# ethz-asl/laser_slam

Measured on NVIDIA H100. Metric: ICP registrations/s (131072-pt scan vs 524288-pt map, 30 iterations), higher is better.
Workload: dtype f32

## Files before the change

laser_slam_b200/csrc/ls_api.cu:

```cuda
#include <cmath>
#include <cstdarg>
#include <cstddef>
#include <cstdio>
#include <cstdlib>
#include <cstring>
#include <string>
#include <utility>
#include <vector>

#include "../../include/ls_b200.h"
#include "ls_filters.cuh"
#include "ls_kernels.cuh"
#include "ls_occupancy.cuh"

using namespace ls;

#define LS_VERSION 100

struct Workspace {
  cudaStream_t stream = nullptr;
  cudaEvent_t ev0 = nullptr, ev1 = nullptr, ev2 = nullptr, ev_launch = nullptr;
  int n_cap = 0, m_cap = 0, cells_cap = 0, tab_cap = 0, hist_cap = 0;
  BuildArrays A{};
  BuildState* bs = nullptr;
  float4* rd = nullptr;
  int* pos = nullptr;
  float4 *vq = nullptr, *vpts = nullptr;
  float* d2 = nullptr;
  int* ids = nullptr;
  float* d2_out = nullptr;
  IcpWork* work = nullptr;
  float* T_hist = nullptr;
  BuildJob* job_host = nullptr;
  BuildJob* job_dev = nullptr;
  IcpWork* h_work = nullptr;
  Grid* h_grid = nullptr;
  IcpProblem hp;
  bool stream_dirty = false;
};

struct ls_ctx {
  int device = 0;
  int sm_count = 0;
  int icp_ctas = 0;
  int icp_ctas_max = 0;
  std::string err;
  uint64_t launches = 0;
  std::vector<Workspace*> ws;
  IcpProblem* probs_dev = nullptr;
  IcpProblem* probs_host = nullptr;
  BuildJob* jobs_dev = nullptr;
  BuildJob* jobs_host = nullptr;
  IcpWork* work_pool = nullptr;
  float4* reading = nullptr;
  float4 *ref_stage = nullptr, *ref_nrm_stage = nullptr;
  int reading_cap = 0, ref_cap = 0;
  float* nrm_raw = nullptr;
  size_t nrm_raw_cap = 0;
  float* T0_dev = nullptr;
  unsigned char* xbuf = nullptr;
  unsigned char* xpeer[8] = {nullptr, nullptr, nullptr, nullptr, nullptr, nullptr, nullptr, nullptr};
  int shard_rank = 0, shard_count = 1;
  bool xconnected = false;
  unsigned int xflag_base = 0;
  bool pending = false;
  int pending_batch = 0;
  std::vector<int> pending_ws;
  std::vector<int> pending_n;
  std::vector<float> pending_T0;
  std::vector<std::pair<const ls_map*, int>> pending_slots;
  lsf::ChainBuffers chain;
};
constexpr int kMaxBatch = 160;

struct ls_scan_slot {
  float4* pts = nullptr;
// ... 180 lines not shown
  const int cap = batch > 1 ? ctx->sm_count * 2 : ctx->sm_count * 8;
  const int pb = blocks_for(m_max, 256, cap);
  reset_build_kernel<<<dim3(1, B), 32, 0, st>>>(jobs_dev);
  LAUNCH_CHECK();
  assemble_kernel<<<dim3(pb, B), 256, 0, st>>>(jobs_dev);
  LAUNCH_CHECK();
  setup_kernel<<<dim3(1, B), 32, 0, st>>>(jobs_dev, r.cell, r.max_cells, r.split);
  LAUNCH_CHECK();
  count0_kernel<<<dim3(pb, B), 256, 0, st>>>(jobs_dev);
  LAUNCH_CHECK();
  const int tiles = (r.max_cells + kScanTile - 1) / kScanTile;
  scan_reduce_kernel<<<dim3(tiles, B), kScanThreads, 0, st>>>(jobs_dev);
  LAUNCH_CHECK();
  scan_apply_kernel<<<dim3(tiles, B), kScanThreads, 0, st>>>(jobs_dev);
  LAUNCH_CHECK();
  pyramid1_kernel<<<dim3(blocks_for(r.max_cells / 16 + 1, 256, batch > 1 ? ctx->sm_count : ctx->sm_count * 4), B), 256, 0, st>>>(jobs_dev);
  LAUNCH_CHECK();
  pyramid_up_kernel<<<dim3(1, B), 1024, 0, st>>>(jobs_dev);
  LAUNCH_CHECK();
  count1_kernel<<<dim3(pb, B), 256, 0, st>>>(jobs_dev);
  LAUNCH_CHECK();
  tables_kernel<<<dim3(cap, B), 256, 0, st>>>(jobs_dev);
  LAUNCH_CHECK();
  scatter_kernel<<<dim3(pb, B), 256, 0, st>>>(jobs_dev);
  LAUNCH_CHECK();
  return LS_OK;
}

int launch_reading_sort(ls_ctx* ctx, const BuildJob* jobs_dev, int batch, int n_max, const Resolved& r, cudaStream_t st) {
  const unsigned int B = (unsigned int)batch;
  const int cap = batch > 1 ? ctx->sm_count * 2 : ctx->sm_count * 8;
  const int qb = blocks_for(n_max, 256, cap);
  const int scan_tiles = (r.max_cells + kScanTile - 1) / kScanTile;
  reading_kernel<<<dim3(qb, B), 256, 0, st>>>(jobs_dev);
  LAUNCH_CHECK();
  q_count_kernel<<<dim3(qb, B), 256, 0, st>>>(jobs_dev);
  LAUNCH_CHECK();
  q_tables_kernel<<<dim3(cap, B), 256, 0, st>>>(jobs_dev);
  LAUNCH_CHECK();
  q_scan_reduce_kernel<<<dim3(scan_tiles, B), kScanThreads, 0, st>>>(jobs_dev);
  LAUNCH_CHECK();
  q_scan_apply_kernel<<<dim3(scan_tiles, B), kScanThreads, 0, st>>>(jobs_dev);
  LAUNCH_CHECK();
  q_scatter_kernel<<<dim3(qb, B), 256, 0, st>>>(jobs_dev);
  LAUNCH_CHECK();
  return LS_OK;
}

int enqueue_build(ls_ctx* ctx, Workspace* w, const Parts& parts, const Resolved& r, const float* T0_host) {
  fill_job(w, parts, T0_host, nullptr, 0);
  CU(cudaMemcpyAsync(w->job_dev, w->job_host, sizeof(BuildJob), cudaMemcpyHostToDevice, w->stream));
  return launch_build(ctx, w->job_dev, 1, w->job_host->m, r, w->stream);
}

int upload_normals(ls_ctx* ctx, Workspace* w, const float* normals, int stride, int n, float4* dst) {
  const size_t need = n > 0 ? (stride <= 8 ? (size_t)(n - 1) * (size_t)stride + 3 : (size_t)n * 3) : 0;
  if (need > ctx->nrm_raw_cap) {
    int rc;
// ... 66 lines not shown
  CU(cudaMemcpyAsync(ctx->probs_dev, ctx->probs_host, sizeof(IcpProblem) * (size_t)batch, cudaMemcpyHostToDevice, w0->stream));
  IcpParamsDev dp;
  dp.max_iterations = prm->max_iterations;
  dp.trim_ratio = prm->trim_ratio;
  dp.use_differential = prm->use_differential;
  dp.min_diff_rot = prm->min_diff_rot;
  dp.min_diff_trans = prm->min_diff_trans;
  dp.smooth_length = prm->smooth_length;
  int ctas = ctx->icp_ctas / batch;
  const int need = (n_max + 31) / 32;
  if (ctas > need) ctas = need;
  if (ctas < 1) ctas = 1;
  const IcpProblem* probs = ctx->probs_dev;
  int dynamic = batch > 1 ? 1 : 0;
  void* args[] = {(void*)&probs, (void*)&ctas, (void*)&dp, (void*)&dynamic};
  if (sharded) {
    shard_slice_kernel<<<1, 32, 0, w0->stream>>>(ctx->probs_dev, w0->job_dev, w0->hp.shard_rank, w0->hp.shard_count);
    LAUNCH_CHECK();
  }
  CU(cudaEventRecord(w0->ev_launch, w0->stream));
  CU(cudaLaunchCooperativeKernel((void*)icp_kernel, dim3(ctas * batch), dim3(kIcpThreads), args, kIcpPairBytes, w0->stream));
  ++ctx->launches;
  CU(cudaEventRecord(w0->ev2, w0->stream));
  for (int b = 0; b < batch; ++b) {
    Workspace* w = ctx->ws[b];
    constexpr size_t off = offsetof(IcpWork, T_out);
    CU(cudaMemcpyAsync(reinterpret_cast<char*>(w->h_work) + off, reinterpret_cast<const char*>(w->work) + off,
                       sizeof(IcpWork) - off, cudaMemcpyDeviceToHost, w0->stream));
    CU(cudaMemcpyAsync(w->h_grid, &w->bs->grid, sizeof(Grid), cudaMemcpyDeviceToHost, w0->stream));
  }
  return LS_OK;
}

int fetch_icp(ls_ctx* ctx, Workspace* w, int n, const float T0[16], float T_out[16], ls_icp_stats* stats,
              bool batch_timing = false) {
  const IcpWork& wk = *w->h_work;
  std::memcpy(T_out, wk.T_out, 16 * sizeof(float));
  if (stats) {
    std::memset(stats, 0, sizeof(*stats));
    stats->iterations = wk.iterations;
    stats->converged = wk.converged;
    stats->max_iter_reached = wk.max_iter_reached;
    stats->last_kept = wk.last_kept;
    stats->last_limit = wk.last_limit;
    stats->used_ratio = n > 0 ? (float)wk.last_kept / (float)n : 0.f;
    float ms = 0.f, bms = 0.f, kms = 0.f;
    const Workspace* tw = batch_timing ? ctx->ws[0] : w;
    cudaEventElapsedTime(&ms, tw->ev0, ctx->ws[0]->ev2);
    cudaEventElapsedTime(&bms, tw->ev0, tw->ev1);
    cudaEventElapsedTime(&kms, ctx->ws[0]->ev_launch, ctx->ws[0]->ev2);
    stats->device_ms = ms;
    stats->build_ms = bms;
    stats->icp_ms = kms;
    stats->grid_cells = w->h_grid->n_cells0;
    stats->grid_tables = w->h_grid->n_tab1;
    stats->grid_overflow = w->h_grid->overflow;
  }
  if (wk.status != 0) {
    std::memcpy(T_out, T0, 16 * sizeof(float));
    return fail(ctx, LS_ERR_CONVERGENCE, "ICP: no point to minimise / non-finite transformation");
  }
  return LS_OK;
}

int run_icp(ls_ctx* ctx, const ls_icp_params* prm, const float4* reading_dev, int n, const float T0[16],
            float T_out[16], ls_icp_stats* stats, int32_t* opt_ids, float* opt_d2, float* opt_T_hist) {
  Workspace* w = ctx->ws[0];
  int rc;
  if ((rc = prep_icp(ctx, w, prm, reading_dev, n, T0, opt_ids || opt_d2, opt_T_hist != nullptr))) return rc;
  if ((rc = launch_icp(ctx, prm, 1, n))) return rc;
  if (opt_ids) CU(cudaMemcpyAsync(opt_ids, w->ids, (size_t)n * sizeof(int), cudaMemcpyDeviceToHost, w->stream));
  if (opt_d2) CU(cudaMemcpyAsync(opt_d2, w->d2_out, (size_t)n * sizeof(float), cudaMemcpyDeviceToHost, w->stream));
  if (opt_T_hist)
    CU(cudaMemcpyAsync(opt_T_hist, w->T_hist, (size_t)prm->max_iterations * 16 * sizeof(float), cudaMemcpyDeviceToHost,
                       w->stream));
  CU(cudaStreamSynchronize(w->stream));
  return fetch_icp(ctx, w, n, T0, T_out, stats);
}

bool is_identity16(const float* T) {
  for (int i = 0; i < 16; ++i)
    if (T[i] != ((i % 5 == 0) ? 1.f : 0.f)) return false;
  return true;
}

const ls_scan_slot* find_slot(const ls_map* map, uint64_t id) {
  const ls_scan_slot& s = map->slots[id % (uint64_t)map->capacity];
  return (s.used && s.id == id) ? &s : nullptr;
}

int wait_slot(const ls_scan_slot* s, cudaStream_t consumer) {
  if (s->async && consumer && cudaStreamWaitEvent(consumer, s->ready, 0) != cudaSuccess) return LS_ERR_CUDA;
  return LS_OK;
}

int make_parts(ls_ctx* ctx, const ls_map* map, int n_parts, const uint64_t* part_ids, const float* T_parts, Parts* out,
               cudaStream_t consumer) {
  if (n_parts < 1 || n_parts > kMaxParts) return fail(ctx, LS_ERR_ARG, "n_parts must be in [1,%d]", kMaxParts);
  Parts& parts = *out;
  std::memset(&parts, 0, sizeof(parts));
// ... 11 lines not shown
    parts.identity[p] = is_identity16(T_parts + 16 * p) ? 1 : 0;
    off += s->n;
    if (off > 0x3fffffff) return fail(ctx, LS_ERR_ARG, "sub-map too large");
  }
  parts.offset[n_parts] = (int)off;
  return LS_OK;
}

}

extern "C" {

int ls_b200_version(void) { return LS_VERSION; }

namespace {
Workspace* new_workspace(ls_ctx* ctx, int index) {
  Workspace* w = new Workspace();
  w->work = ctx->work_pool + index;
  w->job_dev = ctx->jobs_dev + index;
  w->job_host = ctx->jobs_host + index;
  bool ok = cudaStreamCreateWithFlags(&w->stream, cudaStreamNonBlocking) == cudaSuccess &&
            cudaEventCreate(&w->ev0) == cudaSuccess && cudaEventCreate(&w->ev1) == cudaSuccess &&
            cudaEventCreate(&w->ev2) == cudaSuccess && cudaEventCreate(&w->ev_launch) == cudaSuccess &&
            cudaMalloc((void**)&w->bs, sizeof(BuildState)) == cudaSuccess &&
            cudaMallocHost((void**)&w->h_work, sizeof(IcpWork)) == cudaSuccess &&
            cudaMallocHost((void**)&w->h_grid, sizeof(Grid)) == cudaSuccess;
  if (!ok) return nullptr;
  return w;
}
void free_workspace(Workspace* w) {
  if (!w) return;
  if (w->stream) cudaStreamSynchronize(w->stream);
  void* bufs[] = {w->A.sub_pts, w->A.sub_nrm, w->A.srt_pts, w->A.srt_nrm, w->A.pkey, w->A.top, w->A.cnt0, w->A.tab1, w->A.cnt1,
                  w->A.tab1_cell, w->A.pyr, w->A.topmask, w->bs, w->rd, w->pos, w->d2,
                  w->ids, w->vq, w->vpts, w->T_hist, w->d2_out, w->A.qkey, w->A.qperm, w->A.rd_s,
                  w->A.qtab_local, w->A.qtab_total, w->A.qtop_start};
  for (void* b : bufs)
    if (b) cudaFree(b);
  if (w->h_work) cudaFreeHost(w->h_work);
  if (w->h_grid) cudaFreeHost(w->h_grid);
  if (w->ev0) cudaEventDestroy(w->ev0);
  if (w->ev1) cudaEventDestroy(w->ev1);
  if (w->ev2) cudaEventDestroy(w->ev2);
  if (w->ev_launch) cudaEventDestroy(w->ev_launch);
  if (w->stream) cudaStreamDestroy(w->stream);
  delete w;
}
int ensure_workspaces(ls_ctx* ctx, int count) {
  while ((int)ctx->ws.size() < count) {
    Workspace* w = new_workspace(ctx, (int)ctx->ws.size());
    if (!w) return fail(ctx, LS_ERR_NOMEM, "workspace allocation failed");
    ctx->ws.push_back(w);
  }
  return LS_OK;
}
}

int ls_b200_init(int device, ls_ctx** out) {
  if (!out) return LS_ERR_ARG;
  *out = nullptr;
  int count = 0;
  if (cudaGetDeviceCount(&count) != cudaSuccess || count <= 0) return LS_ERR_CUDA;
  if (device < 0 || device >= count) return LS_ERR_ARG;
  ls_ctx* ctx = new ls_ctx();
  ctx->device = device;
  auto bail = [&](int code) {
    ls_b200_destroy(ctx);
    return code;
  };
  if (cudaSetDevice(device) != cudaSuccess) return bail(LS_ERR_CUDA);
  cudaDeviceProp prop;
  if (cudaGetDeviceProperties(&prop, device) != cudaSuccess) return bail(LS_ERR_CUDA);
  if (!prop.cooperativeLaunch) return bail(LS_ERR_CUDA);
  ctx->sm_count = prop.multiProcessorCount;
  int occ = 0;
  if (cudaFuncSetAttribute(icp_kernel, cudaFuncAttributeMaxDynamicSharedMemorySize, kIcpPairBytes) != cudaSuccess ||
      cudaOccupancyMaxActiveBlocksPerMultiprocessor(&occ, icp_kernel, kIcpThreads, kIcpPairBytes) != cudaSuccess || occ < 1)
    return bail(LS_ERR_CUDA);
  ctx->icp_ctas = ctx->icp_ctas_max = occ * ctx->sm_count;
  if (cudaMalloc((void**)&ctx->probs_dev, sizeof(IcpProblem) * kMaxBatch) != cudaSuccess) return bail(LS_ERR_NOMEM);
  if (cudaMallocHost((void**)&ctx->probs_host, sizeof(IcpProblem) * kMaxBatch) != cudaSuccess) return bail(LS_ERR_NOMEM);
  if (cudaMalloc((void**)&ctx->jobs_dev, sizeof(BuildJob) * kMaxBatch) != cudaSuccess) return bail(LS_ERR_NOMEM);
  if (cudaMallocHost((void**)&ctx->jobs_host, sizeof(BuildJob) * kMaxBatch) != cudaSuccess) return bail(LS_ERR_NOMEM);
  if (cudaMalloc((void**)&ctx->work_pool, sizeof(IcpWork) * kMaxBatch) != cudaSuccess) return bail(LS_ERR_NOMEM);
  if (cudaMalloc((void**)&ctx->T0_dev, 16 * sizeof(float)) != cudaSuccess) return bail(LS_ERR_NOMEM);
  if (ensure_workspaces(ctx, 1) != LS_OK) return bail(LS_ERR_NOMEM);
  *out = ctx;
  return LS_OK;
}

void ls_b200_destroy(ls_ctx* ctx) {
  if (!ctx) return;
  cudaSetDevice(ctx->device);
  for (Workspace* w : ctx->ws) free_workspace(w);
  if (ctx->probs_dev) cudaFree(ctx->probs_dev);
  if (ctx->probs_host) cudaFreeHost(ctx->probs_host);
  if (ctx->jobs_dev) cudaFree(ctx->jobs_dev);
  if (ctx->jobs_host) cudaFreeHost(ctx->jobs_host);
  if (ctx->work_pool) cudaFree(ctx->work_pool);
  void* stage[] = {ctx->reading, ctx->ref_stage, ctx->ref_nrm_stage, ctx->nrm_raw, ctx->T0_dev};
  for (void* b : stage)
    if (b) cudaFree(b);
  lsf::release(ctx->chain);
  ls_shard_exchange_close(ctx);
  delete ctx;
}

const char* ls_b200_last_error(const ls_ctx* ctx) { return ctx ? ctx->err.c_str() : "null context"; }
uint64_t ls_b200_launch_count(const ls_ctx* ctx) { return ctx ? ctx->launches : 0; }
int ls_b200_set_icp_cta_budget(ls_ctx* ctx, int ctas) {
  if (!ctx || ctas < 0) return LS_ERR_ARG;
  BUSY_CHECK(ctx);
  ctx->icp_ctas = (ctas == 0 || ctas > ctx->icp_ctas_max) ? ctx->icp_ctas_max : ctas;
  return LS_OK;
}
int ls_b200_icp_cta_budget(const ls_ctx* ctx) { return ctx ? ctx->icp_ctas : LS_ERR_ARG; }

void ls_icp_default_params(ls_icp_params* p) {
  if (!p) return;
  p->max_iterations = 40;
  p->trim_ratio = 0.75f;
  p->use_differential = 1;
// ... 576 lines not shown
  if (n == 0 || m == 0) return fail(ctx, LS_ERR_CONVERGENCE, "empty reading or reference");
  const Resolved r = resolve(prm);
  if ((rc = ensure_capacity(ctx, w, n, m, r.max_cells, prm->max_iterations))) return rc;
  CU(cudaEventRecord(w->ev0, w->stream));
  if ((rc = enqueue_build(ctx, w, parts, r, T0))) return rc;
  if ((rc = prep_icp(ctx, w, prm, rs->pts, n, T0, false, false))) return rc;
  IcpProblem& hp = w->hp;
  hp.shard_rank = shard_rank;
  hp.shard_count = shard_count;
  if (shard_count > 1) {
    IcpWork* slots = reinterpret_cast<IcpWork*>(ctx->xbuf);
    CU(cudaMemsetAsync(slots + shard_rank, 0, sizeof(IcpWork), w->stream));
    hp.link.slots = slots;
    hp.link.flag = reinterpret_cast<unsigned int*>(ctx->xbuf + sizeof(IcpWork) * (size_t)shard_count);
    hp.link.flag_base = ctx->xflag_base;
    for (int g = 0; g < kMaxShards; ++g) {
      unsigned char* pb = g < shard_count ? ctx->xpeer[g] : nullptr;
      hp.link.peer_slots[g] = reinterpret_cast<IcpWork*>(pb);
      hp.link.peer_flag[g] = pb ? reinterpret_cast<unsigned int*>(pb + sizeof(IcpWork) * (size_t)shard_count) : nullptr;
    }
  }
  if ((rc = launch_icp(ctx, prm, 1, 1 << 30, shard_count > 1))) return rc;
  CU(cudaStreamSynchronize(w->stream));
  ctx->xflag_base += w->h_work->xsignals;
  return fetch_icp(ctx, w, n, T0, T_out, stats);
}

int ls_icp_register_submaps(ls_ctx* ctx, const ls_icp_params* prm, const ls_map* ref_map, int n_ref_parts,
                            const uint64_t* ref_part_ids, const float* T_ref_parts, const ls_map* reading_map,
                            int n_reading_parts, const uint64_t* reading_part_ids, const float* T_reading_parts,
                            const float T0[16], float T_out[16], ls_icp_stats* stats) {
  if (!ctx) return LS_ERR_ARG;
  BUSY_CHECK(ctx);
  if (!ref_map || ref_map->ctx != ctx || !reading_map || reading_map->ctx != ctx || !ref_part_ids || !T_ref_parts ||
      !reading_part_ids || !T_reading_parts || !T0 || !T_out)
    return fail(ctx, LS_ERR_ARG, "bad argument");
  int rc = check_params(ctx, prm);
  if (rc) return rc;
  std::memcpy(T_out, T0, 16 * sizeof(float));
  if (stats) std::memset(stats, 0, sizeof(*stats));
  Parts ref, rd;
  CU(cudaSetDevice(ctx->device));
  Workspace* w = ctx->ws[0];
  if ((rc = make_parts(ctx, ref_map, n_ref_parts, ref_part_ids, T_ref_parts, &ref, w->stream))) return rc;
  if ((rc = make_parts(ctx, reading_map, n_reading_parts, reading_part_ids, T_reading_parts, &rd, w->stream))) return rc;
  const int n = rd.offset[n_reading_parts], m = ref.offset[n_ref_parts];
  if (n == 0 || m == 0) return fail(ctx, LS_ERR_CONVERGENCE, "empty reading or reference");
  const Resolved r = resolve(prm);
// ... 75 lines not shown
    ctx->ws[k]->stream_dirty = false;
  }
  CU(cudaEventRecord(w0->ev0, w0->stream));
  CU(cudaMemcpyAsync(ctx->jobs_dev, ctx->jobs_host, sizeof(BuildJob) * (size_t)launched, cudaMemcpyHostToDevice, w0->stream));
  if ((rc = launch_build(ctx, ctx->jobs_dev, launched, m_max, r, w0->stream))) return rc;
  if ((rc = launch_reading_sort(ctx, ctx->jobs_dev, launched, n_max, r, w0->stream))) return rc;
  CU(cudaEventRecord(w0->ev1, w0->stream));
  CU(cudaMemsetAsync(ctx->work_pool, 0, sizeof(IcpWork) * (size_t)launched, w0->stream));
  if ((rc = launch_icp(ctx, prm, launched, n_max))) return rc;
  ctx->pending = true;
  return LS_OK;
}

int ls_icp_register_submap_batch_end(ls_ctx* ctx, float* T_outs, ls_icp_stats* stats, int* statuses) {
  if (!ctx) return LS_ERR_ARG;
  if (!ctx->pending) return fail(ctx, LS_ERR_STATE, "no batch in flight");
  if (!T_outs || !statuses) return fail(ctx, LS_ERR_ARG, "bad argument");
  ctx->pending = false;
  ctx->pending_slots.clear();
  const int batch = ctx->pending_batch;
  std::memcpy(T_outs, ctx->pending_T0.data(), 16 * sizeof(float) * (size_t)batch);
  CU(cudaSetDevice(ctx->device));
  CU(cudaStreamSynchronize(ctx->ws[0]->stream));
  for (int b = 0; b < batch; ++b) {
    const int k = ctx->pending_ws[b];
    if (k < 0) {
      if (stats) std::memset(stats + b, 0, sizeof(*stats));
      statuses[b] = fail(ctx, LS_ERR_CONVERGENCE, "empty reading or reference");
      continue;
    }
    const int st = fetch_icp(ctx, ctx->ws[k], ctx->pending_n[k], ctx->pending_T0.data() + 16 * b, T_outs + 16 * b,
                             stats ? stats + b : nullptr, true);
    if (st < 0) return st;
    statuses[b] = st;
  }
  return LS_OK;
}

int ls_icp_register_submap_batch(ls_ctx* ctx, const ls_icp_params* prm, const ls_map* map, int batch,
                                 const uint64_t* reading_ids, const int* n_parts, const uint64_t* part_ids,
                                 const float* T_parts, const float* T0s, float* T_outs, ls_icp_stats* stats, int* statuses) {
  if (!ctx) return LS_ERR_ARG;
  if (!T_outs || !statuses) return fail(ctx, LS_ERR_ARG, "bad argument");
  if (T0s && batch >= 1 && batch <= kMaxBatch) std::memcpy(T_outs, T0s, 16 * sizeof(float) * (size_t)batch);
  const int rc = ls_icp_register_submap_batch_begin(ctx, prm, map, batch, reading_ids, n_parts, part_ids, T_parts, T0s);
  if (rc != LS_OK) return rc;
  return ls_icp_register_submap_batch_end(ctx, T_outs, stats, statuses);
}

int ls_map_assemble(ls_ctx* ctx, const ls_map* map, int n_parts, const uint64_t* part_ids, const float* T_parts,
                    float* out4, float* out_normals3, int* m_out) {
  if (!ctx) return LS_ERR_ARG;
  BUSY_CHECK(ctx);
  if (!map || map->ctx != ctx || !part_ids || !T_parts || !out4 || !m_out) return fail(ctx, LS_ERR_ARG, "bad argument");
  Parts parts;
// ... 564 lines not shown
```

laser_slam_b200/csrc/ls_kernels.cuh:

```cuda
#pragma once
#include <cuda_runtime.h>
#include <cooperative_groups.h>

#include "ls_grid.cuh"

namespace ls {

constexpr int kMaxParts = 16;
constexpr int kScanTile = 4096;
constexpr int kScanThreads = 512;
constexpr int kIcpThreads = 512;
constexpr int kIcpCtasPerSm = 1024 / kIcpThreads;
constexpr int kMaxSmooth = 15;
constexpr uint32_t kTag1 = 1u << 31, kKeyMask = (1u << 31) - 1u;

struct Parts {
  int n_parts;
  int offset[kMaxParts + 1];
  const float4* pts[kMaxParts];
  const float4* nrm[kMaxParts];
  float T[kMaxParts][16];
  int identity[kMaxParts];
};

struct BuildState {
  unsigned long long sum[3];
  unsigned int minkey[3], maxkey[3];
  Grid grid;
  float T_pre[16];
  unsigned int tile_sums[1024];
};

struct BuildArrays {
  float4* sub_pts;
  float4* sub_nrm;
  float4* srt_pts;
  float4* srt_nrm;
// ... 28 lines not shown
struct IcpParamsDev {
  int max_iterations;
  float trim_ratio;
  int use_differential;
  float min_diff_rot, min_diff_trans;
  int smooth_length;
};

struct alignas(16) IcpWork {
  unsigned int barrier;
  unsigned int pad0[31];
  unsigned int hist[2][5][2048];
  unsigned long long acc[2][32];
  unsigned int qctr[2];
  float T_out[16];
  int status, iterations, converged, max_iter_reached, last_kept;
  float last_limit;
  int fail_code;
  unsigned int xsignals;
  unsigned int dbg_total, dbg_bin[3], dbg_rem[3];
  double dbg_A[6], dbg_x[6];
};

constexpr int kMaxShards = 8;
struct ShardLink {
  IcpWork* slots;
  IcpWork* peer_slots[kMaxShards];
  unsigned int* flag;
  unsigned int* peer_flag[kMaxShards];
  unsigned int flag_base;
};

struct IcpProblem {
  const BuildState* bs;
  GridView view;
  const float4* nrm;
  const float4* rd;
  int n;
  int* pos;
  float* d2;
  int* ids;
  float* d2_out;
  const uint32_t* qperm;
  VLists lists;
  IcpWork* work;
  int shard_rank, shard_count;
// ... 1 lines not shown
  float* T_hist;
  int want_matches;
  unsigned long long* phase_ns;
  float T0[16];
};

__device__ __forceinline__ unsigned int float_order_key(float f) {
  const unsigned int u = __float_as_uint(f);
  return (u & 0x80000000u) ? ~u : (u | 0x80000000u);
}
__device__ __forceinline__ float float_from_order_key(unsigned int k) {
  const unsigned int u = (k & 0x80000000u) ? (k & 0x7fffffffu) : ~k;
  return __uint_as_float(u);
}

__device__ __forceinline__ long long warp_sum_ll(long long v) {
  unsigned int lo = (unsigned int)(v & 0x1FFFFF);
  unsigned int mid = (unsigned int)((v >> 21) & 0x1FFFFF);
  int hi = (int)(v >> 42);
  lo = __reduce_add_sync(0xffffffffu, lo);
  mid = __reduce_add_sync(0xffffffffu, mid);
  hi = __reduce_add_sync(0xffffffffu, hi);
  return ((long long)hi << 42) + ((long long)mid << 21) + (long long)lo;
}

__global__ void __launch_bounds__(256) assemble_kernel(const BuildJob* __restrict__ jobs) {
  const BuildJob& J = jobs[blockIdx.y];
  const Parts& parts = J.parts;
  float4* __restrict__ sub_pts = J.A.sub_pts;
  float4* __restrict__ sub_nrm = J.A.sub_nrm;
  BuildState* bs = J.bs;
  const int total = parts.offset[parts.n_parts];
  long long s0 = 0, s1 = 0, s2 = 0;
  float mn0 = INFINITY, mn1 = INFINITY, mn2 = INFINITY, mx0 = -INFINITY, mx1 = -INFINITY, mx2 = -INFINITY;
  int p = 0;
  for (int i = blockIdx.x * blockDim.x + threadIdx.x; i < total; i += gridDim.x * blockDim.x) {
    while (i >= parts.offset[p + 1]) ++p;
    const int j = i - parts.offset[p];
    float4 a = __ldg(parts.pts[p] + j);
    float4 nn = __ldg(parts.nrm[p] + j);
    if (!parts.identity[p]) {
      float x, y, z;
      xform_point(parts.T[p], a.x, a.y, a.z, x, y, z);
      a.x = x; a.y = y; a.z = z;
      rotate_vec(parts.T[p], nn.x, nn.y, nn.z, x, y, z);
      nn.x = x; nn.y = y; nn.z = z;
// ... 64 lines not shown
  float mu[3], lo[3], hi[3];
  for (int a = 0; a < 3; ++a) {
    const long long s = (long long)bs->sum[a];
    mu[a] = (float)((double)s / ((double)m * 16777216.0));
    lo[a] = float_from_order_key(bs->minkey[a]) - mu[a];
    hi[a] = float_from_order_key(bs->maxkey[a]) - mu[a];
  }
  Grid g;
  grid_setup(g, lo, hi, cell_size, max_cells, leaf_split, m);
  for (int a = 0; a < 3; ++a) g.mu[a] = mu[a];
  bs->grid = g;
  for (int i = 0; i < 16; ++i) bs->T_pre[i] = T0[i];
  for (int a = 0; a < 3; ++a) bs->T_pre[12 + a] = T0[12 + a] - mu[a];
}

__global__ void __launch_bounds__(256) count0_kernel(const BuildJob* __restrict__ jobs) {
  const BuildJob& J = jobs[blockIdx.y];
  const BuildState* __restrict__ bs = J.bs;
  const BuildArrays A = J.A;
  const int m = J.m;
  __shared__ Grid g;
  if (threadIdx.x == 0) g = bs->grid;
  __syncthreads();
  for (int i = blockIdx.x * blockDim.x + threadIdx.x; i < m; i += gridDim.x * blockDim.x) {
    float4 p = A.sub_pts[i];
    p.x = p.x - g.mu[0];
    p.y = p.y - g.mu[1];
    p.z = p.z - g.mu[2];
    A.sub_pts[i] = p;
    const int c0 = top_index(g, p.x, p.y, p.z);
    atomicAdd(&A.cnt0[c0], 1u);
    A.pkey[i] = (uint32_t)c0;
  }
}

__global__ void __launch_bounds__(kScanThreads) scan_reduce_kernel(const BuildJob* __restrict__ jobs) {
  BuildState* bs = jobs[blockIdx.y].bs;
  const uint32_t* __restrict__ cnt0 = jobs[blockIdx.y].A.cnt0;
  const int n = bs->grid.n_cells0;
  const int base = blockIdx.x * kScanTile;
  if (base >= n) return;
  unsigned int s = 0;
  for (int k = threadIdx.x; k < kScanTile; k += kScanThreads) {
    const int c = base + k;
    if (c < n) s += cnt0[c];
  }
  s = __reduce_add_sync(0xffffffffu, s);
  __shared__ unsigned int ws[kScanThreads / 32];
  if ((threadIdx.x & 31) == 0) ws[threadIdx.x >> 5] = s;
  __syncthreads();
  if (threadIdx.x == 0) {
    unsigned int t = 0;
    for (int w = 0; w < kScanThreads / 32; ++w) t += ws[w];
    bs->tile_sums[blockIdx.x] = t;
  }
// ... 97 lines not shown
    A.pyr[g.poff[1] + c] = pyramid_mask(g, 1, x, y, z, A.top, A.pyr);
  }
}

__global__ void __launch_bounds__(1024) pyramid_up_kernel(const BuildJob* __restrict__ jobs) {
  const BuildState* __restrict__ bs = jobs[blockIdx.y].bs;
  const BuildArrays A = jobs[blockIdx.y].A;
  __shared__ Grid g;
  if (threadIdx.x == 0) g = bs->grid;
  __syncthreads();
  for (int l = 2; l <= g.n_pyr; ++l) {
    const int* pd = g.pdim[l];
    const int n = pd[0] * pd[1] * pd[2];
    for (int c = threadIdx.x; c < n; c += blockDim.x) {
      const int x = c % pd[0], y = (c / pd[0]) % pd[1], z = c / (pd[0] * pd[1]);
      A.pyr[g.poff[l] + c] = pyramid_mask(g, l, x, y, z, A.top, A.pyr);
    }
    __threadfence_block();
    __syncthreads();
  }
}

__global__ void __launch_bounds__(256) count1_kernel(const BuildJob* __restrict__ jobs) {
  const BuildState* __restrict__ bs = jobs[blockIdx.y].bs;
  const BuildArrays A = jobs[blockIdx.y].A;
  const int m = jobs[blockIdx.y].m;
  __shared__ Grid g;
  if (threadIdx.x == 0) g = bs->grid;
  __syncthreads();
  for (int i = blockIdx.x * blockDim.x + threadIdx.x; i < m; i += gridDim.x * blockDim.x) {
    const uint32_t c0 = A.pkey[i];
    const Entry e = A.top[c0];
    if (e.meta >= 0) continue;
    const float4 p = A.sub_pts[i];
    float lx, ly, lz;
    top_origin(g, (int)c0, lx, ly, lz);
    const uint32_t key = (uint32_t)(~e.meta) * (uint32_t)LS_FB3 + (uint32_t)sub_index(p.x, p.y, p.z, lx, ly, lz, g.inv1);
    atomicAdd(&A.cnt1[key], 1u);
    A.pkey[i] = kTag1 | key;
  }
}

__global__ void __launch_bounds__(256) tables_kernel(const BuildJob* __restrict__ jobs) {
  BuildState* bs = jobs[blockIdx.y].bs;
  const BuildArrays A = jobs[blockIdx.y].A;
  const int n_tab = min(bs->grid.n_tab1, A.tab_cap);
  constexpr int per = LS_FB3 / 256;
  __shared__ unsigned int ws[8];
  const int lane = threadIdx.x & 31, warp = threadIdx.x >> 5;
  for (int t = blockIdx.x; t < n_tab; t += gridDim.x) {
    const uint32_t* cnt = A.cnt1 + (size_t)t * LS_FB3;
    Entry* tab = A.tab1 + (size_t)t * LS_FB3;
    const uint32_t base = A.top[A.tab1_cell[t]].start;
    unsigned int c[per], loc = 0;
#pragma unroll
    for (int k = 0; k < per; ++k) {
      c[k] = cnt[threadIdx.x * per + k];
      loc += c[k];
    }
    unsigned int incl = loc;
    for (int o = 1; o < 32; o <<= 1) {
// ... 13 lines not shown
      e.meta = (int)c[k];
      tab[threadIdx.x * per + k] = e;
      run += c[k];
    }
    const unsigned int occ = __ballot_sync(0xffffffffu, loc != 0u);
    unsigned int rows8 = 0u;
#pragma unroll
    for (int r = 0; r < 8; ++r)
      if ((occ >> (4 * r)) & 0xFu) rows8 |= 1u << r;
    __syncthreads();
    if (lane == 0) ws[warp] = rows8;
    __syncthreads();
    if (threadIdx.x == 0) {
      unsigned long long m = 0ull;
      for (int w = 0; w < 8; ++w) m |= (unsigned long long)ws[w] << (8 * w);
      A.topmask[A.tab1_cell[t]] = m;
    }
  }
}

__global__ void __launch_bounds__(256) scatter_kernel(const BuildJob* __restrict__ jobs) {
  const BuildArrays A = jobs[blockIdx.y].A;
  const int m = jobs[blockIdx.y].m;
  for (int i = blockIdx.x * blockDim.x + threadIdx.x; i < m; i += gridDim.x * blockDim.x) {
    const uint32_t k = A.pkey[i];
    const uint32_t tag = k & ~kKeyMask, key = k & kKeyMask;
    uint32_t pos;
    if (tag == kTag1) pos = A.tab1[key].start + atomicSub(&A.cnt1[key], 1u) - 1u;
    else pos = A.top[key].start + atomicSub(&A.cnt0[key], 1u) - 1u;
    float4 p = A.sub_pts[i];
    p.w = __int_as_float(i);
    A.srt_pts[pos] = p;
    A.srt_nrm[pos] = A.sub_nrm[i];
  }
}

__global__ void __launch_bounds__(256) q_count_kernel(const BuildJob* __restrict__ jobs) {
  const BuildState* __restrict__ bs = jobs[blockIdx.y].bs;
  const BuildArrays A = jobs[blockIdx.y].A;
  const float4* __restrict__ rd = jobs[blockIdx.y].rd;
  const int n = jobs[blockIdx.y].n;
  __shared__ Grid g;
  if (threadIdx.x == 0) g = bs->grid;
  __syncthreads();
  for (int i = blockIdx.x * blockDim.x + threadIdx.x; i < n; i += gridDim.x * blockDim.x) {
    const float4 p = __ldg(rd + i);
    const int c0 = top_index(g, p.x, p.y, p.z);
    const Entry e = A.top[c0];
    uint32_t key;
    if (e.meta < 0) {
      float lx, ly, lz;
      top_origin(g, c0, lx, ly, lz);
      key = (uint32_t)(~e.meta) * (uint32_t)LS_FB3 + (uint32_t)sub_index(p.x, p.y, p.z, lx, ly, lz, g.inv1);
      atomicAdd(&A.cnt1[key], 1u);
      key |= kTag1;
    } else {
      key = (uint32_t)c0;
      atomicAdd(&A.cnt0[c0], 1u);
    }
    A.qkey[i] = key;
  }
}

__global__ void __launch_bounds__(256) q_tables_kernel(const BuildJob* __restrict__ jobs) {
  BuildState* bs = jobs[blockIdx.y].bs;
  const BuildArrays A = jobs[blockIdx.y].A;
  const int n_tab = min(bs->grid.n_tab1, A.tab_cap);
  constexpr int per = LS_FB3 / 256;
  __shared__ unsigned int ws[8];
  const int lane = threadIdx.x & 31, warp = threadIdx.x >> 5;
  for (int t = blockIdx.x; t < n_tab; t += gridDim.x) {
    const uint32_t* cnt = A.cnt1 + (size_t)t * LS_FB3;
    unsigned int c[per], loc = 0;
#pragma unroll
    for (int k = 0; k < per; ++k) {
      c[k] = cnt[threadIdx.x * per + k];
      loc += c[k];
    }
    unsigned int incl = loc;
    for (int o = 1; o < 32; o <<= 1) {
      const unsigned int v = __shfl_up_sync(0xffffffffu, incl, o);
      if (lane >= o) incl += v;
// ... 73 lines not shown
  unsigned int incl = loc;
  const int lane = threadIdx.x & 31, warp = threadIdx.x >> 5;
  for (int o = 1; o < 32; o <<= 1) {
    const unsigned int v = __shfl_up_sync(0xffffffffu, incl, o);
    if (lane >= o) incl += v;
  }
  __syncthreads();
  if (lane == 31) ws[warp] = incl;
  __syncthreads();
  unsigned int woff = 0;
  for (int w = 0; w < warp; ++w) woff += ws[w];
  unsigned int run = tile_off + woff + incl - loc;
#pragma unroll
  for (int k = 0; k < per; ++k) {
    if (first + k < n) A.qtop_start[first + k] = run;
    run += c[k];
  }
}

__global__ void __launch_bounds__(256) q_scatter_kernel(const BuildJob* __restrict__ jobs) {
  const BuildArrays A = jobs[blockIdx.y].A;
  const float4* __restrict__ rd = jobs[blockIdx.y].rd;
  const int n = jobs[blockIdx.y].n;
  for (int i = blockIdx.x * blockDim.x + threadIdx.x; i < n; i += gridDim.x * blockDim.x) {
    const uint32_t k = A.qkey[i];
    uint32_t rank;
    if (k & kTag1) {
      const uint32_t key = k & kKeyMask;
      rank = A.qtop_start[A.tab1_cell[key / (uint32_t)LS_FB3]] + A.qtab_local[key] + atomicSub(&A.cnt1[key], 1u) - 1u;
    } else {
      rank = A.qtop_start[k] + atomicSub(&A.cnt0[k], 1u) - 1u;
    }
    A.rd_s[rank] = __ldg(rd + i);
    A.qperm[rank] = (uint32_t)i;
  }
}

__global__ void shard_slice_kernel(IcpProblem* P, const BuildJob* __restrict__ job, int shard_rank, int shard_count) {
  if (threadIdx.x != 0 || blockIdx.x != 0) return;
  const BuildArrays A = job->A;
  const int n_cells = job->bs->grid.n_cells0, n = job->n;
  auto cut = [&](int s) -> int {
    if (s <= 0) return 0;
    if (s >= shard_count) return n;
    const unsigned int target = (unsigned int)((long long)n * s / shard_count);
    int lo = 0, hi = n_cells;
    while (lo < hi) {
      const int mid = (lo + hi) >> 1;
      if (A.qtop_start[mid] < target) lo = mid + 1;
      else hi = mid;
    }
    return lo < n_cells ? (int)A.qtop_start[lo] : n;
  };
  const int q0 = cut(shard_rank), q1 = cut(shard_rank + 1);
  P->rd += q0;
  P->qperm += q0;
  P->pos += q0;
  P->d2 += q0;
  P->lists.vq += q0;
  P->lists.vpts += q0;
  P->n = q1 - q0;
}

__global__ void __launch_bounds__(256) reading_kernel(const BuildJob* __restrict__ jobs) {
  const BuildState* __restrict__ bs = jobs[blockIdx.y].bs;
  const float4* __restrict__ in = jobs[blockIdx.y].reading;
  float4* __restrict__ out = jobs[blockIdx.y].rd;
  const int n = jobs[blockIdx.y].n;
  __shared__ float T[16];
  if (threadIdx.x < 16) T[threadIdx.x] = bs->T_pre[threadIdx.x];
  __syncthreads();
  for (int i = blockIdx.x * blockDim.x + threadIdx.x; i < n; i += gridDim.x * blockDim.x) {
    const float4 a = __ldg(in + i);
    float4 o;
    xform_point(T, a.x, a.y, a.z, o.x, o.y, o.z);
    o.w = a.w;
    out[i] = o;
  }
}

__global__ void __launch_bounds__(256) transform_kernel(const float* __restrict__ Tg, const float4* __restrict__ in,
                                                        const float4* __restrict__ nin, int n, float4* __restrict__ out,
                                                        float4* __restrict__ nout) {
  __shared__ float T[16];
  if (threadIdx.x < 16) T[threadIdx.x] = Tg[threadIdx.x];
  __syncthreads();
// ... 2 lines not shown
    float4 o;
    xform_point(T, a.x, a.y, a.z, o.x, o.y, o.z);
    o.w = a.w;
    out[i] = o;
    if (nin) {
      const float4 b = __ldg(nin + i);
      float4 r;
      rotate_vec(T, b.x, b.y, b.z, r.x, r.y, r.z);
      r.w = 0.f;
      nout[i] = r;
    }
  }
}

__global__ void pack_normals_kernel(const float4* __restrict__ in, int n, float* __restrict__ out3) {
  for (int i = blockIdx.x * blockDim.x + threadIdx.x; i < n; i += gridDim.x * blockDim.x) {
    const float4 a = in[i];
    out3[3 * (size_t)i] = a.x;
    out3[3 * (size_t)i + 1] = a.y;
    out3[3 * (size_t)i + 2] = a.z;
  }
}


__global__ void __launch_bounds__(256) nn_query_kernel(const BuildState* __restrict__ bs, GridView view,
                                                       const float4* __restrict__ rd, int n, int* __restrict__ ids,
                                                       float* __restrict__ d2) {
  __shared__ Grid g;
  if (threadIdx.x == 0) g = bs->grid;
  __syncthreads();
  for (int i = blockIdx.x * blockDim.x + threadIdx.x; i < n; i += gridDim.x * blockDim.x) {
    const float4 q = __ldg(rd + i);
    const Best b = nn_search(g, view, q.x, q.y, q.z, -1, INFINITY);
    ids[i] = b.idx;
    d2[i] = b.d2;
  }
}

__global__ void __launch_bounds__(128) knn_normals_kernel(const BuildState* __restrict__ bs, GridView view,
                                                           const float4* __restrict__ pts_c ,
                                                           int n, int k, float4* __restrict__ out) {
  __shared__ Grid g;
  if (threadIdx.x == 0) g = bs->grid;
  __syncthreads();
  for (int i = blockIdx.x * blockDim.x + threadIdx.x; i < n; i += gridDim.x * blockDim.x) {
    const float4 q = __ldg(pts_c + i);
    TopK t;
    knn_search(g, view, q.x, q.y, q.z, k, t);
    int cnt = 0;
    double mx = 0.0, my = 0.0, mz = 0.0;
    for (int j = 0; j < k; ++j) {
      if (t.id[j] == INT_MAX) break;
      const float4 p = __ldg(pts_c + t.id[j]);
      mx = mx + (double)p.x;
      my = my + (double)p.y;
      mz = mz + (double)p.z;
      ++cnt;
    }
    float4 nn = make_float4(0.f, 0.f, 0.f, 0.f);
    if (cnt >= 3) {
      const double inv = 1.0 / (double)cnt;
      mx = mx * inv; my = my * inv; mz = mz * inv;
      double C[9] = {0, 0, 0, 0, 0, 0, 0, 0, 0};
      for (int j = 0; j < cnt; ++j) {
        const float4 p = __ldg(pts_c + t.id[j]);
        const double dx = (double)p.x - mx, dy = (double)p.y - my, dz = (double)p.z - mz;
        C[0] = C[0] + dx * dx; C[1] = C[1] + dx * dy; C[2] = C[2] + dx * dz;
        C[4] = C[4] + dy * dy; C[5] = C[5] + dy * dz; C[8] = C[8] + dz * dz;
      }
      C[3] = C[1]; C[6] = C[2]; C[7] = C[5];
      double nv[3];
      smallest_eigvec3(C, nv);
      const double ox = (double)q.x + (double)g.mu[0], oy = (double)q.y + (double)g.mu[1], oz = (double)q.z + (double)g.mu[2];
      const double dot = nv[0] * ox + (nv[1] * oy + nv[2] * oz);
      const double sgn = dot > 0.0 ? -1.0 : 1.0;
      nn = make_float4((float)(sgn * nv[0]), (float)(sgn * nv[1]), (float)(sgn * nv[2]), 0.f);
    }
    out[i] = nn;
  }
}

__device__ __forceinline__ unsigned long long globaltimer_ns() {
  unsigned long long t;
  asm volatile("mov.u64 %0, %%globaltimer;" : "=l"(t));
  return t;
}
#define LS_STAMP(slot)                                                                   \
  do {                                                                                   \
// ... 632 lines not shown
```

Measured before the change: 942.0.

## Aggregate grid-build atomics per warp, fuse reading transform, gather ICP results

Several build and readback changes go in together. Per-point atomic counting and ranking in the count and scatter kernels now uses warp-level match_any aggregation, so one leader atomic serves each group of equal keys. The sub-cell index is packed into the key during count0, so count1 no longer reloads points. Map centring moves into scatter, and knn_normals now centres points when it reads them. The reading transform is fused into q_count, which drops a kernel launch, and per-problem result copies are replaced by one gather kernel and a single device-to-host copy. The costs are more complex key packing (a 22-bit cell limit) and sub_pts is no longer centred in place, which any other reader of sub_pts must now handle.

```diff
diff --git a/laser_slam_b200/csrc/ls_api.cu b/laser_slam_b200/csrc/ls_api.cu
--- a/laser_slam_b200/csrc/ls_api.cu
+++ b/laser_slam_b200/csrc/ls_api.cu
@@ -33,8 +33,6 @@
   float* T_hist = nullptr;
   BuildJob* job_host = nullptr;
   BuildJob* job_dev = nullptr;
-  IcpWork* h_work = nullptr;
-  Grid* h_grid = nullptr;
   IcpProblem hp;
   bool stream_dirty = false;
 };
@@ -52,6 +50,8 @@
   BuildJob* jobs_dev = nullptr;
   BuildJob* jobs_host = nullptr;
   IcpWork* work_pool = nullptr;
+  IcpResult* results_dev = nullptr;
+  IcpResult* results_host = nullptr;
   float4* reading = nullptr;
   float4 *ref_stage = nullptr, *ref_nrm_stage = nullptr;
   int reading_cap = 0, ref_cap = 0;
@@ -278,7 +278,7 @@
   LAUNCH_CHECK();
   tables_kernel<<<dim3(cap, B), 256, 0, st>>>(jobs_dev);
   LAUNCH_CHECK();
-  scatter_kernel<<<dim3(pb, B), 256, 0, st>>>(jobs_dev);
+  scatter_kernel<<<dim3(blocks_for(m_max, 256, ctx->sm_count * 16), B), 256, 0, st>>>(jobs_dev);
   LAUNCH_CHECK();
   return LS_OK;
 }
@@ -288,8 +288,6 @@
   const int cap = batch > 1 ? ctx->sm_count * 2 : ctx->sm_count * 8;
   const int qb = blocks_for(n_max, 256, cap);
   const int scan_tiles = (r.max_cells + kScanTile - 1) / kScanTile;
-  reading_kernel<<<dim3(qb, B), 256, 0, st>>>(jobs_dev);
-  LAUNCH_CHECK();
   q_count_kernel<<<dim3(qb, B), 256, 0, st>>>(jobs_dev);
   LAUNCH_CHECK();
   q_tables_kernel<<<dim3(cap, B), 256, 0, st>>>(jobs_dev);
@@ -402,19 +400,24 @@
   CU(cudaLaunchCooperativeKernel((void*)icp_kernel, dim3(ctas * batch), dim3(kIcpThreads), args, kIcpPairBytes, w0->stream));
   ++ctx->launches;
   CU(cudaEventRecord(w0->ev2, w0->stream));
-  for (int b = 0; b < batch; ++b) {
-    Workspace* w = ctx->ws[b];
-    constexpr size_t off = offsetof(IcpWork, T_out);
-    CU(cudaMemcpyAsync(reinterpret_cast<char*>(w->h_work) + off, reinterpret_cast<const char*>(w->work) + off,
-                       sizeof(IcpWork) - off, cudaMemcpyDeviceToHost, w0->stream));
-    CU(cudaMemcpyAsync(w->h_grid, &w->bs->grid, sizeof(Grid), cudaMemcpyDeviceToHost, w0->stream));
-  }
-  return LS_OK;
-}
-
-int fetch_icp(ls_ctx* ctx, Workspace* w, int n, const float T0[16], float T_out[16], ls_icp_stats* stats,
-              bool batch_timing = false) {
-  const IcpWork& wk = *w->h_work;
+  collect_results_kernel<<<batch, 32, 0, w0->stream>>>(ctx->probs_dev, ctx->results_dev);
+  LAUNCH_CHECK();
+  CU(cudaMemcpyAsync(ctx->results_host, ctx->results_dev, sizeof(IcpResult) * (size_t)batch, cudaMemcpyDeviceToHost,
+                     w0->stream));
+  return LS_OK;
+}
+
+void launch_times(ls_ctx* ctx, float t[3]) {
+  const Workspace* w = ctx->ws[0];
+  t[0] = t[1] = t[2] = 0.f;
+  cudaEventElapsedTime(&t[0], w->ev0, w->ev2);
+  cudaEventElapsedTime(&t[1], w->ev0, w->ev1);
+  cudaEventElapsedTime(&t[2], w->ev_launch, w->ev2);
+}
+
+int fetch_icp(ls_ctx* ctx, int k, int n, const float T0[16], float T_out[16], ls_icp_stats* stats,
+              const float* times = nullptr) {
+  const IcpResult& wk = ctx->results_host[k];
   std::memcpy(T_out, wk.T_out, 16 * sizeof(float));
   if (stats) {
     std::memset(stats, 0, sizeof(*stats));
@@ -424,17 +427,17 @@
     stats->last_kept = wk.last_kept;
     stats->last_limit = wk.last_limit;
     stats->used_ratio = n > 0 ? (float)wk.last_kept / (float)n : 0.f;
-    float ms = 0.f, bms = 0.f, kms = 0.f;
-    const Workspace* tw = batch_timing ? ctx->ws[0] : w;
-    cudaEventElapsedTime(&ms, tw->ev0, ctx->ws[0]->ev2);
-    cudaEventElapsedTime(&bms, tw->ev0, tw->ev1);
-    cudaEventElapsedTime(&kms, ctx->ws[0]->ev_launch, ctx->ws[0]->ev2);
-    stats->device_ms = ms;
-    stats->build_ms = bms;
-    stats->icp_ms = kms;
-    stats->grid_cells = w->h_grid->n_cells0;
-    stats->grid_tables = w->h_grid->n_tab1;
-    stats->grid_overflow = w->h_grid->overflow;
+    float own[3];
+    if (!times) {
+      launch_times(ctx, own);
+      times = own;
+    }
+    stats->device_ms = times[0];
+    stats->build_ms = times[1];
+    stats->icp_ms = times[2];
+    stats->grid_cells = wk.n_cells0;
+    stats->grid_tables = wk.n_tab1;
+    stats->grid_overflow = wk.overflow;
   }
   if (wk.status != 0) {
     std::memcpy(T_out, T0, 16 * sizeof(float));
@@ -455,7 +458,7 @@
     CU(cudaMemcpyAsync(opt_T_hist, w->T_hist, (size_t)prm->max_iterations * 16 * sizeof(float), cudaMemcpyDeviceToHost,
                        w->stream));
   CU(cudaStreamSynchronize(w->stream));
-  return fetch_icp(ctx, w, n, T0, T_out, stats);
+  return fetch_icp(ctx, 0, n, T0, T_out, stats);
 }
 
 bool is_identity16(const float* T) {
@@ -513,9 +516,7 @@
   bool ok = cudaStreamCreateWithFlags(&w->stream, cudaStreamNonBlocking) == cudaSuccess &&
             cudaEventCreate(&w->ev0) == cudaSuccess && cudaEventCreate(&w->ev1) == cudaSuccess &&
             cudaEventCreate(&w->ev2) == cudaSuccess && cudaEventCreate(&w->ev_launch) == cudaSuccess &&
-            cudaMalloc((void**)&w->bs, sizeof(BuildState)) == cudaSuccess &&
-            cudaMallocHost((void**)&w->h_work, sizeof(IcpWork)) == cudaSuccess &&
-            cudaMallocHost((void**)&w->h_grid, sizeof(Grid)) == cudaSuccess;
+            cudaMalloc((void**)&w->bs, sizeof(BuildState)) == cudaSuccess;
   if (!ok) return nullptr;
   return w;
 }
@@ -528,8 +529,6 @@
                   w->A.qtab_local, w->A.qtab_total, w->A.qtop_start};
   for (void* b : bufs)
     if (b) cudaFree(b);
-  if (w->h_work) cudaFreeHost(w->h_work);
-  if (w->h_grid) cudaFreeHost(w->h_grid);
   if (w->ev0) cudaEventDestroy(w->ev0);
   if (w->ev1) cudaEventDestroy(w->ev1);
   if (w->ev2) cudaEventDestroy(w->ev2);
@@ -574,6 +573,8 @@
   if (cudaMalloc((void**)&ctx->jobs_dev, sizeof(BuildJob) * kMaxBatch) != cudaSuccess) return bail(LS_ERR_NOMEM);
   if (cudaMallocHost((void**)&ctx->jobs_host, sizeof(BuildJob) * kMaxBatch) != cudaSuccess) return bail(LS_ERR_NOMEM);
   if (cudaMalloc((void**)&ctx->work_pool, sizeof(IcpWork) * kMaxBatch) != cudaSuccess) return bail(LS_ERR_NOMEM);
+  if (cudaMalloc((void**)&ctx->results_dev, sizeof(IcpResult) * kMaxBatch) != cudaSuccess) return bail(LS_ERR_NOMEM);
+  if (cudaMallocHost((void**)&ctx->results_host, sizeof(IcpResult) * kMaxBatch) != cudaSuccess) return bail(LS_ERR_NOMEM);
   if (cudaMalloc((void**)&ctx->T0_dev, 16 * sizeof(float)) != cudaSuccess) return bail(LS_ERR_NOMEM);
   if (ensure_workspaces(ctx, 1) != LS_OK) return bail(LS_ERR_NOMEM);
   *out = ctx;
@@ -589,6 +590,8 @@
   if (ctx->jobs_dev) cudaFree(ctx->jobs_dev);
   if (ctx->jobs_host) cudaFreeHost(ctx->jobs_host);
   if (ctx->work_pool) cudaFree(ctx->work_pool);
+  if (ctx->results_dev) cudaFree(ctx->results_dev);
+  if (ctx->results_host) cudaFreeHost(ctx->results_host);
   void* stage[] = {ctx->reading, ctx->ref_stage, ctx->ref_nrm_stage, ctx->nrm_raw, ctx->T0_dev};
   for (void* b : stage)
     if (b) cudaFree(b);
@@ -1211,8 +1214,8 @@
   }
   if ((rc = launch_icp(ctx, prm, 1, 1 << 30, shard_count > 1))) return rc;
   CU(cudaStreamSynchronize(w->stream));
-  ctx->xflag_base += w->h_work->xsignals;
-  return fetch_icp(ctx, w, n, T0, T_out, stats);
+  ctx->xflag_base += ctx->results_host[0].xsignals;
+  return fetch_icp(ctx, 0, n, T0, T_out, stats);
 }
 
 int ls_icp_register_submaps(ls_ctx* ctx, const ls_icp_params* prm, const ls_map* ref_map, int n_ref_parts,
@@ -1334,6 +1337,8 @@
   std::memcpy(T_outs, ctx->pending_T0.data(), 16 * sizeof(float) * (size_t)batch);
   CU(cudaSetDevice(ctx->device));
   CU(cudaStreamSynchronize(ctx->ws[0]->stream));
+  float times[3] = {0.f, 0.f, 0.f};
+  if (stats && !ctx->pending_n.empty()) launch_times(ctx, times);
   for (int b = 0; b < batch; ++b) {
     const int k = ctx->pending_ws[b];
     if (k < 0) {
@@ -1341,8 +1346,8 @@
       statuses[b] = fail(ctx, LS_ERR_CONVERGENCE, "empty reading or reference");
       continue;
     }
-    const int st = fetch_icp(ctx, ctx->ws[k], ctx->pending_n[k], ctx->pending_T0.data() + 16 * b, T_outs + 16 * b,
-                             stats ? stats + b : nullptr, true);
+    const int st = fetch_icp(ctx, k, ctx->pending_n[k], ctx->pending_T0.data() + 16 * b, T_outs + 16 * b,
+                             stats ? stats + b : nullptr, times);
     if (st < 0) return st;
     statuses[b] = st;
   }
diff --git a/laser_slam_b200/csrc/ls_kernels.cuh b/laser_slam_b200/csrc/ls_kernels.cuh
--- a/laser_slam_b200/csrc/ls_kernels.cuh
+++ b/laser_slam_b200/csrc/ls_kernels.cuh
@@ -13,6 +13,8 @@
 constexpr int kIcpCtasPerSm = 1024 / kIcpThreads;
 constexpr int kMaxSmooth = 15;
 constexpr uint32_t kTag1 = 1u << 31, kKeyMask = (1u << 31) - 1u;
+constexpr int kSubShift = 22;
+constexpr uint32_t kCellMask = (1u << kSubShift) - 1u;
 
 struct Parts {
   int n_parts;
@@ -87,6 +89,14 @@
   double dbg_A[6], dbg_x[6];
 };
 
+struct IcpResult {
+  float T_out[16];
+  int status, iterations, converged, max_iter_reached, last_kept;
+  float last_limit;
+  unsigned int xsignals;
+  int n_cells0, n_tab1, overflow;
+};
+
 constexpr int kMaxShards = 8;
 struct ShardLink {
   IcpWork* slots;
@@ -134,6 +144,20 @@
   mid = __reduce_add_sync(0xffffffffu, mid);
   hi = __reduce_add_sync(0xffffffffu, hi);
   return ((long long)hi << 42) + ((long long)mid << 21) + (long long)lo;
+}
+
+__device__ __forceinline__ void warp_count(uint32_t* ctr, uint32_t key, unsigned int active) {
+  const unsigned int peers = __match_any_sync(active, key);
+  if ((threadIdx.x & 31) == (unsigned int)(__ffs(peers) - 1)) atomicAdd(ctr, (unsigned int)__popc(peers));
+}
+__device__ __forceinline__ uint32_t warp_take(uint32_t* ctr, uint32_t key, unsigned int active) {
+  const unsigned int peers = __match_any_sync(active, key);
+  const int leader = __ffs(peers) - 1;
+  const unsigned int lane = threadIdx.x & 31;
+  uint32_t old = 0;
+  if (lane == (unsigned int)leader) old = atomicSub(ctr, (unsigned int)__popc(peers));
+  old = __shfl_sync(peers, old, leader);
+  return old - 1u - (uint32_t)__popc(peers & ((1u << lane) - 1u));
 }
 
 __global__ void __launch_bounds__(256) assemble_kernel(const BuildJob* __restrict__ jobs) {
@@ -244,15 +268,17 @@
   __shared__ Grid g;
   if (threadIdx.x == 0) g = bs->grid;
   __syncthreads();
-  for (int i = blockIdx.x * blockDim.x + threadIdx.x; i < m; i += gridDim.x * blockDim.x) {
-    float4 p = A.sub_pts[i];
-    p.x = p.x - g.mu[0];
-    p.y = p.y - g.mu[1];
-    p.z = p.z - g.mu[2];
-    A.sub_pts[i] = p;
-    const int c0 = top_index(g, p.x, p.y, p.z);
-    atomicAdd(&A.cnt0[c0], 1u);
-    A.pkey[i] = (uint32_t)c0;
+  const int lane = threadIdx.x & 31;
+  for (int i = blockIdx.x * blockDim.x + threadIdx.x; i - lane < m; i += gridDim.x * blockDim.x) {
+    const unsigned int active = __ballot_sync(0xffffffffu, i < m);
+    if (i >= m) break;
+    const float4 p = A.sub_pts[i];
+    const float x = p.x - g.mu[0], y = p.y - g.mu[1], z = p.z - g.mu[2];
+    const int c0 = top_index(g, x, y, z);
+    float lx, ly, lz;
+    top_origin(g, c0, lx, ly, lz);
+    warp_count(A.cnt0 + c0, (uint32_t)c0, active);
+    A.pkey[i] = ((uint32_t)sub_index(x, y, z, lx, ly, lz, g.inv1) << kSubShift) | (uint32_t)c0;
   }
 }
 
@@ -396,21 +422,16 @@
 }
 
 __global__ void __launch_bounds__(256) count1_kernel(const BuildJob* __restrict__ jobs) {
-  const BuildState* __restrict__ bs = jobs[blockIdx.y].bs;
   const BuildArrays A = jobs[blockIdx.y].A;
   const int m = jobs[blockIdx.y].m;
-  __shared__ Grid g;
-  if (threadIdx.x == 0) g = bs->grid;
-  __syncthreads();
-  for (int i = blockIdx.x * blockDim.x + threadIdx.x; i < m; i += gridDim.x * blockDim.x) {
-    const uint32_t c0 = A.pkey[i];
-    const Entry e = A.top[c0];
-    if (e.meta >= 0) continue;
-    const float4 p = A.sub_pts[i];
-    float lx, ly, lz;
-    top_origin(g, (int)c0, lx, ly, lz);
-    const uint32_t key = (uint32_t)(~e.meta) * (uint32_t)LS_FB3 + (uint32_t)sub_index(p.x, p.y, p.z, lx, ly, lz, g.inv1);
-    atomicAdd(&A.cnt1[key], 1u);
+  const int lane = threadIdx.x & 31;
+  for (int i = blockIdx.x * blockDim.x + threadIdx.x; i - lane < m; i += gridDim.x * blockDim.x) {
+    const uint32_t k = i < m ? A.pkey[i] : 0u;
+    const int meta = i < m ? A.top[k & kCellMask].meta : 0;
+    const unsigned int active = __ballot_sync(0xffffffffu, meta < 0);
+    if (meta >= 0) continue;
+    const uint32_t key = (uint32_t)(~meta) * (uint32_t)LS_FB3 + (k >> kSubShift);
+    warp_count(A.cnt1 + key, key, active);
     A.pkey[i] = kTag1 | key;
   }
 }
@@ -470,13 +491,22 @@
 __global__ void __launch_bounds__(256) scatter_kernel(const BuildJob* __restrict__ jobs) {
   const BuildArrays A = jobs[blockIdx.y].A;
   const int m = jobs[blockIdx.y].m;
-  for (int i = blockIdx.x * blockDim.x + threadIdx.x; i < m; i += gridDim.x * blockDim.x) {
+  const float* mu = jobs[blockIdx.y].bs->grid.mu;
+  const float mx = mu[0], my = mu[1], mz = mu[2];
+  const int lane = threadIdx.x & 31;
+  for (int i = blockIdx.x * blockDim.x + threadIdx.x; i - lane < m; i += gridDim.x * blockDim.x) {
+    const unsigned int active = __ballot_sync(0xffffffffu, i < m);
+    if (i >= m) break;
     const uint32_t k = A.pkey[i];
-    const uint32_t tag = k & ~kKeyMask, key = k & kKeyMask;
-    uint32_t pos;
-    if (tag == kTag1) pos = A.tab1[key].start + atomicSub(&A.cnt1[key], 1u) - 1u;
-    else pos = A.top[key].start + atomicSub(&A.cnt0[key], 1u) - 1u;
+    const bool fine = (k & kTag1) != 0u;
+    const uint32_t key = fine ? k : (k & kCellMask);
+    const Entry* e = fine ? A.tab1 + (key & kKeyMask) : A.top + key;
+    uint32_t* ctr = fine ? A.cnt1 + (key & kKeyMask) : A.cnt0 + key;
+    const uint32_t pos = e->start + warp_take(ctr, key, active);
     float4 p = A.sub_pts[i];
+    p.x = p.x - mx;
+    p.y = p.y - my;
+    p.z = p.z - mz;
     p.w = __int_as_float(i);
     A.srt_pts[pos] = p;
     A.srt_nrm[pos] = A.sub_nrm[i];
@@ -486,26 +516,38 @@
 __global__ void __launch_bounds__(256) q_count_kernel(const BuildJob* __restrict__ jobs) {
   const BuildState* __restrict__ bs = jobs[blockIdx.y].bs;
   const BuildArrays A = jobs[blockIdx.y].A;
-  const float4* __restrict__ rd = jobs[blockIdx.y].rd;
+  const float4* __restrict__ in = jobs[blockIdx.y].reading;
+  float4* __restrict__ rd = jobs[blockIdx.y].rd;
   const int n = jobs[blockIdx.y].n;
   __shared__ Grid g;
+  __shared__ float T[16];
   if (threadIdx.x == 0) g = bs->grid;
-  __syncthreads();
-  for (int i = blockIdx.x * blockDim.x + threadIdx.x; i < n; i += gridDim.x * blockDim.x) {
-    const float4 p = __ldg(rd + i);
+  if (threadIdx.x < 16) T[threadIdx.x] = bs->T_pre[threadIdx.x];
+  __syncthreads();
+  const int lane = threadIdx.x & 31;
+  for (int i = blockIdx.x * blockDim.x + threadIdx.x; i - lane < n; i += gridDim.x * blockDim.x) {
+    const unsigned int active = __ballot_sync(0xffffffffu, i < n);
+    if (i >= n) break;
+    const float4 a = __ldg(in + i);
+    float4 p;
+    xform_point(T, a.x, a.y, a.z, p.x, p.y, p.z);
+    p.w = a.w;
+    rd[i] = p;
     const int c0 = top_index(g, p.x, p.y, p.z);
     const Entry e = A.top[c0];
     uint32_t key;
+    uint32_t* ctr;
     if (e.meta < 0) {
       float lx, ly, lz;
       top_origin(g, c0, lx, ly, lz);
       key = (uint32_t)(~e.meta) * (uint32_t)LS_FB3 + (uint32_t)sub_index(p.x, p.y, p.z, lx, ly, lz, g.inv1);
-      atomicAdd(&A.cnt1[key], 1u);
+      ctr = A.cnt1 + key;
       key |= kTag1;
     } else {
       key = (uint32_t)c0;
-      atomicAdd(&A.cnt0[c0], 1u);
-    }
+      ctr = A.cnt0 + c0;
+    }
+    warp_count(ctr, key, active);
     A.qkey[i] = key;
   }
 }
@@ -625,15 +667,22 @@
   const BuildArrays A = jobs[blockIdx.y].A;
   const float4* __restrict__ rd = jobs[blockIdx.y].rd;
   const int n = jobs[blockIdx.y].n;
-  for (int i = blockIdx.x * blockDim.x + threadIdx.x; i < n; i += gridDim.x * blockDim.x) {
+  const int lane = threadIdx.x & 31;
+  for (int i = blockIdx.x * blockDim.x + threadIdx.x; i - lane < n; i += gridDim.x * blockDim.x) {
+    const unsigned int active = __ballot_sync(0xffffffffu, i < n);
+    if (i >= n) break;
     const uint32_t k = A.qkey[i];
-    uint32_t rank;
+    uint32_t start;
+    uint32_t* ctr;
     if (k & kTag1) {
       const uint32_t key = k & kKeyMask;
-      rank = A.qtop_start[A.tab1_cell[key / (uint32_t)LS_FB3]] + A.qtab_local[key] + atomicSub(&A.cnt1[key], 1u) - 1u;
+      start = A.qtop_start[A.tab1_cell[key / (uint32_t)LS_FB3]] + A.qtab_local[key];
+      ctr = A.cnt1 + key;
     } else {
-      rank = A.qtop_start[k] + atomicSub(&A.cnt0[k], 1u) - 1u;
-    }
+      start = A.qtop_start[k];
+      ctr = A.cnt0 + k;
+    }
+    const uint32_t rank = start + warp_take(ctr, k, active);
     A.rd_s[rank] = __ldg(rd + i);
     A.qperm[rank] = (uint32_t)i;
   }
@@ -665,6 +714,25 @@
   P->n = q1 - q0;
 }
 
+__global__ void collect_results_kernel(const IcpProblem* __restrict__ probs, IcpResult* __restrict__ out) {
+  const IcpProblem& P = probs[blockIdx.x];
+  const IcpWork* W = P.work;
+  IcpResult& r = out[blockIdx.x];
+  if (threadIdx.x < 16) r.T_out[threadIdx.x] = W->T_out[threadIdx.x];
+  if (threadIdx.x == 0) {
+    r.status = W->status;
+    r.iterations = W->iterations;
+    r.converged = W->converged;
+    r.max_iter_reached = W->max_iter_reached;
+    r.last_kept = W->last_kept;
+    r.last_limit = W->last_limit;
+    r.xsignals = W->xsignals;
+    r.n_cells0 = P.bs->grid.n_cells0;
+    r.n_tab1 = P.bs->grid.n_tab1;
+    r.overflow = P.bs->grid.overflow;
+  }
+}
+
 __global__ void __launch_bounds__(256) reading_kernel(const BuildJob* __restrict__ jobs) {
   const BuildState* __restrict__ bs = jobs[blockIdx.y].bs;
   const float4* __restrict__ in = jobs[blockIdx.y].reading;
@@ -713,7 +781,6 @@
   }
 }
 
-
 __global__ void __launch_bounds__(256) nn_query_kernel(const BuildState* __restrict__ bs, GridView view,
                                                        const float4* __restrict__ rd, int n, int* __restrict__ ids,
                                                        float* __restrict__ d2) {
@@ -729,20 +796,27 @@
 }
 
 __global__ void __launch_bounds__(128) knn_normals_kernel(const BuildState* __restrict__ bs, GridView view,
-                                                           const float4* __restrict__ pts_c ,
+                                                           const float4* __restrict__ pts ,
                                                            int n, int k, float4* __restrict__ out) {
   __shared__ Grid g;
   if (threadIdx.x == 0) g = bs->grid;
   __syncthreads();
+  auto centred = [&](int j) {
+    float4 p = __ldg(pts + j);
+    p.x = p.x - g.mu[0];
+    p.y = p.y - g.mu[1];
+    p.z = p.z - g.mu[2];
+    return p;
+  };
   for (int i = blockIdx.x * blockDim.x + threadIdx.x; i < n; i += gridDim.x * blockDim.x) {
-    const float4 q = __ldg(pts_c + i);
+    const float4 q = centred(i);
     TopK t;
     knn_search(g, view, q.x, q.y, q.z, k, t);
     int cnt = 0;
     double mx = 0.0, my = 0.0, mz = 0.0;
     for (int j = 0; j < k; ++j) {
       if (t.id[j] == INT_MAX) break;
-      const float4 p = __ldg(pts_c + t.id[j]);
+      const float4 p = centred(t.id[j]);
       mx = mx + (double)p.x;
       my = my + (double)p.y;
       mz = mz + (double)p.z;
@@ -754,7 +828,7 @@
       mx = mx * inv; my = my * inv; mz = mz * inv;
       double C[9] = {0, 0, 0, 0, 0, 0, 0, 0, 0};
       for (int j = 0; j < cnt; ++j) {
-        const float4 p = __ldg(pts_c + t.id[j]);
+        const float4 p = centred(t.id[j]);
         const double dx = (double)p.x - mx, dy = (double)p.y - my, dz = (double)p.z - mz;
         C[0] = C[0] + dx * dx; C[1] = C[1] + dx * dy; C[2] = C[2] + dx * dz;
         C[4] = C[4] + dy * dy; C[5] = C[5] + dy * dz; C[8] = C[8] + dz * dz;
```

Measured after the change: 984.3, median of 6. +4.5%, better.
